# lxa9867/ImageFolder

Hardware: NVIDIA H100
Metric: tokenizer_train_images_per_sec_256x256 (higher is better)
Workload: dtype bf16

## Files before the change

imagefolder_b200/csrc/attn_kernel.cu:

```cuda
#include "xq_common.cuh"
#include "xq_tc.cuh"

namespace xq {
using namespace xqtc;

constexpr int AT_BM = 128;
constexpr int AT_BN = 128;
constexpr int AT_D = 64;
constexpr int AT_NS = 2;
constexpr int AT_TILE = AT_BM * AT_D * 2;
constexpr int AT_THREADS = 288;

struct AttnFwdSmem {
    static constexpr int Q = 0;
    static constexpr int K = AT_TILE;
    static constexpr int V = AT_TILE * (1 + AT_NS);
    static constexpr int BAR = AT_TILE * (1 + 2 * AT_NS);
    static constexpr int BYTES = BAR + 256;
};

__device__ __forceinline__ void named_bar_sync(int id, int nthreads) { asm volatile("bar.sync %0, %1;" ::"r"(id), "r"(nthreads) : "memory"); }

__global__ void __launch_bounds__(AT_THREADS, 1)
attn_fwd_kernel(const __grid_constant__ CUtensorMap tmQKV, __nv_bfloat16 *__restrict__ out, float *__restrict__ lse2, int N, int H,
                int nQ , float c ) {
    extern __shared__ uint8_t smem_raw[];
    uint8_t *base = (uint8_t *)(((uintptr_t)smem_raw + 1023) & ~(uintptr_t)1023);
    uint64_t *bars = (uint64_t *)(base + AttnFwdSmem::BAR);
    uint64_t *q_full = bars + 0;
    uint64_t *k_full = bars + 1;
    uint64_t *k_empty = bars + 1 + AT_NS;
    uint64_t *v_full = bars + 1 + 2 * AT_NS;
    uint64_t *v_empty = bars + 1 + 3 * AT_NS;

    const int tid = threadIdx.x, warp = tid >> 5, lane = tid & 31;
    const int nK = (N + AT_BN - 1) / AT_BN;
    const int bh = blockIdx.x / nQ, qt = blockIdx.x - bh * nQ;
    const int b = bh / H, h = bh - b * H;

    if (tid == 0) {
        mbar_init(q_full, 1);
        for (int i = 0; i < AT_NS; ++i) { mbar_init(&k_full[i], 1); mbar_init(&k_empty[i], 8); mbar_init(&v_full[i], 1); mbar_init(&v_empty[i], 8); }
        mbar_fence_init();
    }
    __syncthreads();

    if (warp == 8) {
        const int colQ = h * AT_D, colK = (H + h) * AT_D, colV = (2 * H + h) * AT_D;
        if (elect_one()) {
            tma_prefetch_desc(&tmQKV);
            mbar_expect_tx(q_full, AT_TILE);
            tma_load_3d(base + AttnFwdSmem::Q, &tmQKV, colQ, qt * AT_BM, b, q_full);
        }
        __syncwarp();
        for (int j = 0; j < nK; ++j) {
            const int st = j % AT_NS;
            const uint32_t ph = ((j / AT_NS) & 1) ^ 1;
            mbar_wait(&k_empty[st], ph);
            if (elect_one()) {
                mbar_expect_tx(&k_full[st], AT_TILE);
                tma_load_3d(base + AttnFwdSmem::K + st * AT_TILE, &tmQKV, colK, j * AT_BN, b, &k_full[st]);
            }
            __syncwarp();
            mbar_wait(&v_empty[st], ph);
            if (elect_one()) {
                mbar_expect_tx(&v_full[st], AT_TILE);
                tma_load_3d(base + AttnFwdSmem::V + st * AT_TILE, &tmQKV, colV, j * AT_BN, b, &v_full[st]);
            }
            __syncwarp();
        }
        return;
    }

    const int wg = warp >> 2, wq = warp & 3;
    const int rq = wg * 64 + wq * 16 + (lane >> 2), cq = 2 * (lane & 3);
    const uint64_t qd = desc_k_sw128(smem_u32(base + AttnFwdSmem::Q + wg * (AT_TILE / 2)));
    float m[2] = {-CUDART_INF_F, -CUDART_INF_F}, l[2] = {0.f, 0.f};
    float o[32];
#pragma unroll
    for (int i = 0; i < 32; ++i) o[i] = 0.f;
    mbar_wait(q_full, 0);
    for (int j = 0; j < nK; ++j) {
        const int st = j % AT_NS;
        const uint32_t ph = (j / AT_NS) & 1;
        float s[64];
        mbar_wait(&k_full[st], ph);
        const uint64_t kd = desc_k_sw128(smem_u32(base + AttnFwdSmem::K + st * AT_TILE));
        wgmma_fence();
#pragma unroll
        for (int k = 0; k < AT_D / 16; ++k) wgmma_m64n128k16_ss<0, 0>(s, desc_adv(qd, k * 32), desc_adv(kd, k * 32), (uint32_t)k);
        wgmma_commit();
        wgmma_wait<0>();
        fence_regs(s);
        __syncwarp();
        if (lane == 0) mbar_arrive(&k_empty[st]);
        const int nv = N - j * AT_BN;
        if (nv < AT_BN) {
#pragma unroll
            for (int i = 0; i < 64; ++i)
                if (8 * (i >> 2) + cq + (i & 1) >= nv) s[i] = -CUDART_INF_F;
        }
        float mx[2] = {m[0], m[1]};
#pragma unroll
        for (int i = 0; i < 64; ++i) mx[(i >> 1) & 1] = fmaxf(mx[(i >> 1) & 1], s[i]);
// ... 53 lines not shown

__global__ void __launch_bounds__(128)
attn_fwd_tail_kernel(const __nv_bfloat16 *__restrict__ qkv, __nv_bfloat16 *__restrict__ out, float *__restrict__ lse2, int B, int N,
                     int H, int n0 , float c) {
    const int lane = threadIdx.x & 31;
    const long long w = ((long long)blockIdx.x * blockDim.x + threadIdx.x) >> 5;
    const int nt = N - n0;
    if (w >= (long long)B * H * nt) return;
    const int r = (int)(w % nt);
    const int bh = (int)(w / nt);
    const int b = bh / H, h = bh - b * H;
    const int n = n0 + r;
    const size_t W = (size_t)3 * H * AT_D;
    const __nv_bfloat16 *qp = qkv + ((size_t)b * N + n) * W + h * AT_D;
    float qf[AT_D];
#pragma unroll
    for (int u = 0; u < 8; ++u) {
        const uint4 x = *reinterpret_cast<const uint4 *>(qp + u * 8);
        const __nv_bfloat162 *x2 = reinterpret_cast<const __nv_bfloat162 *>(&x);
#pragma unroll
        for (int e = 0; e < 4; ++e) {
            const float2 f = __bfloat1622float2(x2[e]);
            qf[u * 8 + 2 * e] = f.x * c;
            qf[u * 8 + 2 * e + 1] = f.y * c;
        }
    }
    float m = -CUDART_INF_F, l = 0.f, o[AT_D];
#pragma unroll
    for (int i = 0; i < AT_D; ++i) o[i] = 0.f;
    for (int key = lane; key < N; key += 32) {
        const __nv_bfloat16 *kp = qkv + ((size_t)b * N + key) * W + (H + h) * AT_D;
        const __nv_bfloat16 *vp = kp + (size_t)H * AT_D;
        float s = 0.f;
#pragma unroll
        for (int u = 0; u < 8; ++u) {
            const uint4 x = *reinterpret_cast<const uint4 *>(kp + u * 8);
            const __nv_bfloat162 *x2 = reinterpret_cast<const __nv_bfloat162 *>(&x);
#pragma unroll
            for (int e = 0; e < 4; ++e) {
                const float2 f = __bfloat1622float2(x2[e]);
                s = fmaf(qf[u * 8 + 2 * e], f.x, s);
                s = fmaf(qf[u * 8 + 2 * e + 1], f.y, s);
            }
        }
        const float m_new = fmaxf(m, s);
        const float corr = ex2_approx(m - m_new);
        const float p = ex2_approx(s - m_new);
        l = fmaf(l, corr, p);
        m = m_new;
#pragma unroll
        for (int u = 0; u < 8; ++u) {
            const uint4 x = *reinterpret_cast<const uint4 *>(vp + u * 8);
            const __nv_bfloat162 *x2 = reinterpret_cast<const __nv_bfloat162 *>(&x);
#pragma unroll
            for (int e = 0; e < 4; ++e) {
                const float2 f = __bfloat1622float2(x2[e]);
                o[u * 8 + 2 * e] = fmaf(o[u * 8 + 2 * e], corr, p * f.x);
                o[u * 8 + 2 * e + 1] = fmaf(o[u * 8 + 2 * e + 1], corr, p * f.y);
            }
        }
    }
    float M = m;
#pragma unroll
    for (int off = 16; off > 0; off >>= 1) M = fmaxf(M, __shfl_xor_sync(0xffffffffu, M, off));
    const float f = (m == -CUDART_INF_F) ? 0.f : ex2_approx(m - M);
    l *= f;
#pragma unroll
    for (int off = 16; off > 0; off >>= 1) l += __shfl_xor_sync(0xffffffffu, l, off);
    const float inv = 1.0f / l;
    float mine0 = 0.f, mine1 = 0.f;
#pragma unroll
    for (int i = 0; i < AT_D; ++i) {
        float x = o[i] * f;
#pragma unroll
        for (int off = 16; off > 0; off >>= 1) x += __shfl_xor_sync(0xffffffffu, x, off);
        if (i == 2 * lane) mine0 = x;
        if (i == 2 * lane + 1) mine1 = x;
    }
    __nv_bfloat16 *op = out + ((size_t)b * N + n) * H * AT_D + h * AT_D;
    *reinterpret_cast<uint32_t *>(op + 2 * lane) = pack_bf16(mine0 * inv, mine1 * inv);
    if (lane == 0) lse2[(size_t)bh * N + n] = M + log2f(l);
}

constexpr int AB_THREADS = 288;
constexpr int AB_BQ = 64;
constexpr int AB_QS = 3;
constexpr int AB_QTILE = AB_BQ * AT_D * 2;

struct AttnBwdSmem {
    static constexpr int K = 0;
    static constexpr int V = AT_TILE;
    static constexpr int Q = 2 * AT_TILE;
    static constexpr int DO = Q + AB_QS * AB_QTILE;
    static constexpr int DS = DO + AB_QS * AB_QTILE;
    static constexpr int STAT = DS + 2 * AB_QTILE;
    static constexpr int BAR = STAT + AB_QS * 512;
    static constexpr int BYTES = BAR + 256;
};

__device__ __forceinline__ void bwd_epilogue_frag(const float (&acc)[32], float mul, __nv_bfloat16 *__restrict__ row0,
                                                  size_t row_stride, bool ok0, bool ok1, float *__restrict__ g_bias_cols, int lane) {
    const int cq = 2 * (lane & 3);
#pragma unroll
    for (int jj = 0; jj < AT_D / 8; ++jj) {
        const uint32_t w0 = pack_bf16(acc[4 * jj] * mul, acc[4 * jj + 1] * mul);
        const uint32_t w1 = pack_bf16(acc[4 * jj + 2] * mul, acc[4 * jj + 3] * mul);
        if (ok0) *reinterpret_cast<uint32_t *>(row0 + 8 * jj + cq) = w0;
        if (ok1) *reinterpret_cast<uint32_t *>(row0 + 8 * row_stride + 8 * jj + cq) = w1;
        if (g_bias_cols) {
            float s0 = __uint_as_float(w0 << 16) + __uint_as_float(w1 << 16);
            float s1 = __uint_as_float(w0 & 0xffff0000u) + __uint_as_float(w1 & 0xffff0000u);
#pragma unroll
            for (int o = 4; o < 32; o <<= 1) {
                s0 += __shfl_xor_sync(0xffffffffu, s0, o);
                s1 += __shfl_xor_sync(0xffffffffu, s1, o);
            }
            if (lane < 4) {
                atomicAdd(g_bias_cols + 8 * jj + cq, s0);
                atomicAdd(g_bias_cols + 8 * jj + cq + 1, s1);
            }
        }
    }
}

__global__ void __launch_bounds__(AB_THREADS, 1)
attn_bwd_kernel(const __grid_constant__ CUtensorMap tmQKV, const __grid_constant__ CUtensorMap tmDO, const float *__restrict__ lseP,
                const float *__restrict__ deltaP, float *__restrict__ dq_acc, __nv_bfloat16 *__restrict__ dqkv, float *__restrict__ g_bias,
                int N, int H, int Npad, float c, float scale) {
    extern __shared__ uint8_t smem_raw[];
    uint8_t *base = (uint8_t *)(((uintptr_t)smem_raw + 1023) & ~(uintptr_t)1023);
    uint64_t *bars = (uint64_t *)(base + AttnBwdSmem::BAR);
    uint64_t *kv_full = bars;
    uint64_t *q_full = bars + 1;
    uint64_t *q_empty = bars + 1 + AB_QS;
    float *s_lse = (float *)(base + AttnBwdSmem::STAT);
    float *s_delta = s_lse + AB_QS * AB_BQ;

    const int tid = threadIdx.x, warp = tid >> 5, lane = tid & 31;
    const int bh = blockIdx.y, b = bh / H, h = bh - b * H;
    const int k0 = blockIdx.x * AT_BN;
    const int colQ = h * AT_D, colK = (H + h) * AT_D, colV = (2 * H + h) * AT_D;
    const int nQ = (N + AB_BQ - 1) / AB_BQ;

    if (tid == 0) {
        mbar_init(kv_full, 1);
        for (int i = 0; i < AB_QS; ++i) { mbar_init(&q_full[i], 1); mbar_init(&q_empty[i], 8); }
        mbar_fence_init();
    }
    __syncthreads();

    if (warp == 8) {
        if (elect_one()) {
            tma_prefetch_desc(&tmQKV);
            tma_prefetch_desc(&tmDO);
            mbar_expect_tx(kv_full, 2 * AT_TILE);
            for (int hf = 0; hf < 2; ++hf) {
                tma_load_3d(base + AttnBwdSmem::K + hf * AB_QTILE, &tmQKV, colK, k0 + hf * AB_BQ, b, kv_full);
                tma_load_3d(base + AttnBwdSmem::V + hf * AB_QTILE, &tmQKV, colV, k0 + hf * AB_BQ, b, kv_full);
            }
        }
        __syncwarp();
        for (int i = 0; i < nQ; ++i) {
            const int st = i % AB_QS;
            mbar_wait(&q_empty[st], ((i / AB_QS) & 1) ^ 1);
            if (elect_one()) {
                mbar_expect_tx(&q_full[st], 2 * AB_QTILE + 2 * AB_BQ * 4);
                tma_load_3d(base + AttnBwdSmem::Q + st * AB_QTILE, &tmQKV, colQ, i * AB_BQ, b, &q_full[st]);
                tma_load_3d(base + AttnBwdSmem::DO + st * AB_QTILE, &tmDO, h * AT_D, i * AB_BQ, b, &q_full[st]);
                bulk_g2s(s_lse + st * AB_BQ, lseP + (size_t)bh * Npad + i * AB_BQ, AB_BQ * 4, &q_full[st]);
                bulk_g2s(s_delta + st * AB_BQ, deltaP + (size_t)bh * Npad + i * AB_BQ, AB_BQ * 4, &q_full[st]);
            }
            __syncwarp();
        }
        return;
    }

    const int wg = warp >> 2, wq = warp & 3;
    const int rq = wq * 16 + (lane >> 2), cq = 2 * (lane & 3);
    const int key0 = k0 + wg * 64 + rq;
    const bool kok0 = key0 < N, kok1 = key0 + 8 < N;
    const uint32_t kw = smem_u32(base + AttnBwdSmem::K + wg * AB_QTILE), vw = smem_u32(base + AttnBwdSmem::V + wg * AB_QTILE);
    const uint64_t kd_k = desc_k_sw128(kw), vd_k = desc_k_sw128(vw), kd_mn = desc_mn_sw128(kw, AT_TILE);
    const uint32_t dsw = smem_u32(base + AttnBwdSmem::DS + wg * AB_QTILE);
    const uint64_t dsd = desc_mn_sw128(dsw, AT_TILE);
    float dv[32], dk[32];
#pragma unroll
    for (int i = 0; i < 32; ++i) dv[i] = dk[i] = 0.f;
    mbar_wait(kv_full, 0);
    for (int i = 0; i < nQ; ++i) {
        const int st = i % AB_QS;
        mbar_wait(&q_full[st], (i / AB_QS) & 1);
        const uint32_t qa = smem_u32(base + AttnBwdSmem::Q + st * AB_QTILE), da = smem_u32(base + AttnBwdSmem::DO + st * AB_QTILE);
        float s[32], dp[32];
        wgmma_fence();
#pragma unroll
        for (int k = 0; k < AT_D / 16; ++k) wgmma_m64n64k16_ss<0, 0>(s, desc_adv(kd_k, k * 32), desc_adv(desc_k_sw128(qa), k * 32), (uint32_t)k);
#pragma unroll
        for (int k = 0; k < AT_D / 16; ++k) wgmma_m64n64k16_ss<0, 0>(dp, desc_adv(vd_k, k * 32), desc_adv(desc_k_sw128(da), k * 32), (uint32_t)k);
        wgmma_commit();
        wgmma_wait<0>();
        fence_regs(s);
        fence_regs(dp);
        const float *L = s_lse + st * AB_BQ, *D = s_delta + st * AB_BQ;
        uint32_t pa[4][4], sa[4][4];
#pragma unroll
        for (int jj = 0; jj < AB_BQ / 8; ++jj) {
            const float2 Lq = *reinterpret_cast<const float2 *>(L + 8 * jj + cq);
            const float2 Dq = *reinterpret_cast<const float2 *>(D + 8 * jj + cq);
#pragma unroll
            for (int hh = 0; hh < 2; ++hh) {
                const bool ok = hh ? kok1 : kok0;
                const float p0 = ok ? ex2_approx(fmaf(s[4 * jj + 2 * hh], c, -Lq.x)) : 0.f;
                const float p1 = ok ? ex2_approx(fmaf(s[4 * jj + 2 * hh + 1], c, -Lq.y)) : 0.f;
                const uint32_t pw = pack_bf16(p0, p1);
                const float d0 = __uint_as_float(pw << 16) * (dp[4 * jj + 2 * hh] - Dq.x);
                const float d1 = __uint_as_float(pw & 0xffff0000u) * (dp[4 * jj + 2 * hh + 1] - Dq.y);
                const uint32_t dw = pack_bf16(d0, d1);
                pa[jj >> 1][(jj & 1) * 2 + hh] = pw;
                sa[jj >> 1][(jj & 1) * 2 + hh] = dw;
                asm volatile("st.shared.b32 [%0], %1;" ::"r"(dsw + rowtile_off_bf16(rq + 8 * hh, 8 * jj + cq)), "r"(dw) : "memory");
            }
        }
        fence_async_smem();
        named_bar_sync(1 + wg, 128);
        const uint64_t qd_mn = desc_mn_sw128(qa, AT_TILE), dd_mn = desc_mn_sw128(da, AT_TILE);
        float dq[32];
        wgmma_fence();
#pragma unroll
        for (int k = 0; k < AB_BQ / 16; ++k) {
            wgmma_m64n64k16_rs<1>(dv, pa[k], desc_adv(dd_mn, k * 2048), 1u);
            wgmma_m64n64k16_rs<1>(dk, sa[k], desc_adv(qd_mn, k * 2048), 1u);
        }
#pragma unroll
        for (int k = 0; k < 64 / 16; ++k) wgmma_m64n64k16_ss<1, 1>(dq, desc_adv(dsd, k * 2048), desc_adv(kd_mn, k * 2048), (uint32_t)k);
        wgmma_commit();
        wgmma_wait<0>();
        fence_regs(dv);
        fence_regs(dk);
        fence_regs(dq);
        __syncwarp();
        if (lane == 0) mbar_arrive(&q_empty[st]);
        named_bar_sync(1 + wg, 128);
#pragma unroll
        for (int hh = 0; hh < 2; ++hh) {
            const int q = i * AB_BQ + rq + 8 * hh;
            if (q < N) {
                float *dst = dq_acc + ((size_t)bh * N + q) * AT_D + cq;
#pragma unroll
                for (int jj = 0; jj < AT_D / 8; ++jj)
                    atomicAdd(reinterpret_cast<float2 *>(dst + 8 * jj), make_float2(dq[4 * jj + 2 * hh], dq[4 * jj + 2 * hh + 1]));
            }
        }
    }
    const size_t W = (size_t)3 * H * AT_D;
    __nv_bfloat16 *row = dqkv + ((size_t)b * N + key0) * W;
    bwd_epilogue_frag(dv, 1.0f, row + colV, W, kok0, kok1, g_bias ? g_bias + colV : nullptr, lane);
    bwd_epilogue_frag(dk, scale, row + colK, W, kok0, kok1, g_bias ? g_bias + colK : nullptr, lane);
}


constexpr int AB_KTAIL_MAX = 4;
constexpr int AB_PREP_ROWS = 128;

__device__ __forceinline__ void unpack8(const uint4 &w, float (&f)[8]) {
    const uint32_t x[4] = {w.x, w.y, w.z, w.w};
#pragma unroll
    for (int e = 0; e < 4; ++e) { f[2 * e] = __uint_as_float(x[e] << 16); f[2 * e + 1] = __uint_as_float(x[e] & 0xffff0000u); }
}

template <int NT>
__global__ void __launch_bounds__(256, 2)
attn_bwd_prep_kernel(const __nv_bfloat16 *__restrict__ qkv, const __nv_bfloat16 *__restrict__ out, const __nv_bfloat16 *__restrict__ dout,
                     const float *__restrict__ lse2, float *__restrict__ lseP, float *__restrict__ deltaP, float *__restrict__ dq_acc,
                     float *__restrict__ dsT, __nv_bfloat16 *__restrict__ dqkv, float *__restrict__ g_bias, int N, int H, int Npad,
                     float c, float scale) {
    constexpr int NTA = NT > 0 ? NT : 1;
    __shared__ float red[NT > 0 ? 8 : 1][2][NTA][AT_D];
    __shared__ __align__(16) float skv[2][NTA][AT_D];
    const int bh = blockIdx.y, b = bh / H, h = bh - b * H;
    const int lane = threadIdx.x & 31, sub = threadIdx.x & 7, rloc = threadIdx.x >> 3;
    const int n0 = N - NT;
    const size_t W = (size_t)3 * H * AT_D;
    const __nv_bfloat16 *qb = qkv + (size_t)b * N * W + h * AT_D + sub * 8;
    const size_t ob = (size_t)b * N * H * AT_D + h * AT_D + sub * 8;
    float aK[NTA][8], aV[NTA][8];
    if constexpr (NT > 0) {
        if (threadIdx.x < NT * 16) {
            const int t = threadIdx.x >> 4, isv = (threadIdx.x >> 3) & 1;
            float f[8];
            unpack8(*reinterpret_cast<const uint4 *>(qb + (size_t)(n0 + t) * W + (size_t)(1 + isv) * H * AT_D), f);
#pragma unroll
            for (int e = 0; e < 8; ++e) skv[isv][t][sub * 8 + e] = f[e];
        }
#pragma unroll
        for (int t = 0; t < NT; ++t) {
#pragma unroll
            for (int e = 0; e < 8; ++e) aK[t][e] = aV[t][e] = 0.f;
        }
        __syncthreads();
    }
    constexpr int PASSES = AB_PREP_ROWS / 32;
    extern __shared__ uint4 prep_stage[];
    auto prefetch = [&](int blk, int stg) {
#pragma unroll
        for (int ps = 0; ps < PASSES; ++ps) {
            const int n = blk * AB_PREP_ROWS + ps * 32 + rloc;
            const int nc = n < N ? n : N - 1;
            uint4 *dst = prep_stage + ((size_t)(stg * 3) * PASSES + ps) * 256 + threadIdx.x;
            cp_async16(dst, out + ob + (size_t)nc * H * AT_D);
            cp_async16(dst + PASSES * 256, dout + ob + (size_t)nc * H * AT_D);
            cp_async16(dst + 2 * PASSES * 256, qb + (size_t)nc * W);
        }
        cp_async_commit();
    };
    if constexpr (NT > 0) prefetch(blockIdx.x, 0);
    int stg = 0;
    for (int blk = blockIdx.x; blk * AB_PREP_ROWS < Npad; blk += gridDim.x, stg ^= 1) {
        uint4 ow[PASSES], gw[PASSES], qw[PASSES];
        float lq[PASSES];
#pragma unroll
        for (int ps = 0; ps < PASSES; ++ps) {
            const int n = blk * AB_PREP_ROWS + ps * 32 + rloc;
            const int nc = n < N ? n : N - 1;
            if constexpr (NT == 0) {
                ow[ps] = *reinterpret_cast<const uint4 *>(out + ob + (size_t)nc * H * AT_D);
                gw[ps] = *reinterpret_cast<const uint4 *>(dout + ob + (size_t)nc * H * AT_D);
            }
            lq[ps] = lse2[(size_t)bh * N + nc];
        }
        if constexpr (NT > 0) {
            if ((blk + (int)gridDim.x) * AB_PREP_ROWS < Npad) { prefetch(blk + gridDim.x, stg ^ 1); cp_async_wait<1>(); }
            else cp_async_wait<0>();
        }
#pragma unroll
        for (int ps = 0; ps < PASSES; ++ps) {
            const int n = blk * AB_PREP_ROWS + ps * 32 + rloc;
// ... 109 lines not shown
    for (int e = 0; e < 8; ++e) v[e] = 0.f;
#pragma unroll
    for (int ps = 0; ps < PASSES; ++ps) {
        const int n = blockIdx.x * AB_CONV_ROWS + ps * 32 + rloc;
        if (n < N) {
            const size_t rowid = (size_t)bhh * N + n;
            float x[8] = {x0[ps].x, x0[ps].y, x0[ps].z, x0[ps].w, x1[ps].x, x1[ps].y, x1[ps].z, x1[ps].w};
            for (int t = 0; t < nt; ++t) {
                const float ds = dsT[rowid * nt + t];
#pragma unroll
                for (int e = 0; e < 8; ++e) x[e] = fmaf(ds, skt[t][part * 8 + e], x[e]);
            }
            uint4 o;
            o.x = pack_bf16(x[0] * scale, x[1] * scale);
            o.y = pack_bf16(x[2] * scale, x[3] * scale);
            o.z = pack_bf16(x[4] * scale, x[5] * scale);
            o.w = pack_bf16(x[6] * scale, x[7] * scale);
            *reinterpret_cast<uint4 *>(dqkv + (((size_t)bb * N + n) * 3 * H + hh) * AT_D + part * 8) = o;
            const uint32_t w[4] = {o.x, o.y, o.z, o.w};
#pragma unroll
            for (int e = 0; e < 4; ++e) { v[2 * e] += __uint_as_float(w[e] << 16); v[2 * e + 1] += __uint_as_float(w[e] & 0xffff0000u); }
        }
    }
    if (!g_bias) return;
#pragma unroll
    for (int e = 0; e < 8; ++e) {
        v[e] += __shfl_xor_sync(0xffffffffu, v[e], 8);
        v[e] += __shfl_xor_sync(0xffffffffu, v[e], 16);
    }
    const int warp = threadIdx.x >> 5, lane = threadIdx.x & 31;
    if (lane < 8) {
#pragma unroll
        for (int e = 0; e < 8; ++e) red[warp][lane * 8 + e] = v[e];
    }
    __syncthreads();
    if (threadIdx.x < AT_D) {
        float acc = 0.f;
#pragma unroll
        for (int w8 = 0; w8 < 8; ++w8) acc += red[w8][threadIdx.x];
        atomicAdd(g_bias + hh * AT_D + threadIdx.x, acc);
    }
}

static int attn_bwd_ktail(int N) {
    const int r = N % AT_BN;
    return (N > AT_BN && r != 0 && r <= AB_KTAIL_MAX) ? r : 0;
}

static size_t attn_bwd_ws_layout(int B, int N, int H, size_t *off_lse, size_t *off_delta, size_t *off_dst) {
    const size_t Npad = ((size_t)N + AT_BM - 1) / AT_BM * AT_BM;
    const size_t acc = align_up((size_t)B * H * N * AT_D * sizeof(float), 1024);
    const size_t st = align_up((size_t)B * H * Npad * sizeof(float), 1024);
    const size_t dst = align_up((size_t)B * H * N * attn_bwd_ktail(N) * sizeof(float), 1024);
    if (off_lse) *off_lse = acc;
    if (off_delta) *off_delta = acc + st;
    if (off_dst) *off_dst = acc + 2 * st;
    return acc + 2 * st + dst;
}

}

extern "C" {

size_t xq_vit_attn_bwd_workspace_bytes(int B, int N, int H) {
    if (B <= 0 || N <= 0 || H <= 0) return 0;
    return xq::attn_bwd_ws_layout(B, N, H, nullptr, nullptr, nullptr);
}

int xq_vit_attn_bwd(const void *qkv, const void *out, const void *d_out, const float *lse2, void *dqkv, float *g_bias, int B, int N,
                    int H, int head_dim, float scale, void *workspace, size_t workspace_bytes, void *stream) {
    using namespace xq;
    if (!qkv || !out || !d_out || !lse2 || !dqkv || !workspace || B <= 0 || N <= 0 || H <= 0) return XQ_ERR_ARG;
    if (head_dim != AT_D) return XQ_ERR_UNSUPPORTED;
    if (((uintptr_t)qkv & 15) || ((uintptr_t)out & 15) || ((uintptr_t)d_out & 15) || ((uintptr_t)dqkv & 15) || ((uintptr_t)workspace & 255))
        return XQ_ERR_ARG;
    size_t off_lse, off_delta, off_dst;
    if (workspace_bytes < attn_bwd_ws_layout(B, N, H, &off_lse, &off_delta, &off_dst)) return XQ_ERR_WORKSPACE;
    cudaStream_t st = (cudaStream_t)stream;
    float *acc = (float *)workspace;
    float *lseP = (float *)((char *)workspace + off_lse);
    float *deltaP = (float *)((char *)workspace + off_delta);
    float *dsT = (float *)((char *)workspace + off_dst);
    const uint64_t W = (uint64_t)3 * H * AT_D, Wo = (uint64_t)H * AT_D;
    CUtensorMap tmQKV, tmDO;
    if (!tensor_map_bf16_3d(&tmQKV, qkv, W, N, B, W * 2, (uint64_t)N * W * 2, AB_BQ) ||
        !tensor_map_bf16_3d(&tmDO, d_out, Wo, N, B, Wo * 2, (uint64_t)N * Wo * 2, AB_BQ))
        return XQ_ERR_UNSUPPORTED;
    const int nt = attn_bwd_ktail(N);
    const int nK = nt ? N / AT_BN : (N + AT_BN - 1) / AT_BN;
    const int Npad = (N + AT_BM - 1) / AT_BM * AT_BM;
    if ((long long)B * H > 65535) return XQ_ERR_UNSUPPORTED;
    if (g_bias) XQ_CUDA_TRY(cudaMemsetAsync(g_bias, 0, (size_t)3 * H * AT_D * sizeof(float), st));
    const float c2 = scale * 1.4426950408889634f;
    {
        dim3 grid(nt ? 1u : (unsigned)(Npad / AB_PREP_ROWS), (unsigned)(B * H));
        const size_t ps = nt ? (size_t)2 * 3 * (AB_PREP_ROWS / 32) * 256 * 16 : 0;
        decltype(&attn_bwd_prep_kernel<0>) const preps[] = {attn_bwd_prep_kernel<0>, attn_bwd_prep_kernel<1>, attn_bwd_prep_kernel<2>,
                                                            attn_bwd_prep_kernel<3>, attn_bwd_prep_kernel<4>};
        const auto prep = preps[nt < 4 ? nt : 4];
        if (int rc = smem_optin(prep, ps)) return rc;
        prep<<<grid, 256, ps, st>>>((const __nv_bfloat16 *)qkv, (const __nv_bfloat16 *)out, (const __nv_bfloat16 *)d_out, lse2, lseP,
                                    deltaP, acc, dsT, (__nv_bfloat16 *)dqkv, g_bias, N, H, Npad, c2, scale);
        XQ_LAUNCH_CHECK("attn_bwd_prep_kernel");
    }
    const size_t smem = AttnBwdSmem::BYTES + 1024;
    if (int rc = smem_optin(attn_bwd_kernel, smem)) return rc;
    attn_bwd_kernel<<<dim3((unsigned)nK, (unsigned)(B * H)), AB_THREADS, smem, st>>>(tmQKV, tmDO, lseP, deltaP, acc,
                                                                                     (__nv_bfloat16 *)dqkv, g_bias, N, H, Npad, c2, scale);
    XQ_LAUNCH_CHECK("attn_bwd_kernel");
    {
        dim3 grid((unsigned)((N + AB_CONV_ROWS - 1) / AB_CONV_ROWS), (unsigned)(B * H));
        attn_dq_convert_kernel<<<grid, 256, 0, st>>>(acc, (const __nv_bfloat16 *)qkv, dsT, (__nv_bfloat16 *)dqkv, g_bias, N, H, N - nt, nt, scale);
        XQ_LAUNCH_CHECK("attn_dq_convert_kernel");
    }
    return XQ_OK;
}

int xq_vit_attn_fwd(const void *qkv, void *out, float *lse2, int B, int N, int H, int head_dim, float scale, void *stream) {
    using namespace xq;
    if (!qkv || !out || !lse2 || B <= 0 || N <= 0 || H <= 0) return XQ_ERR_ARG;
    if (head_dim != AT_D) return XQ_ERR_UNSUPPORTED;
    if (((uintptr_t)qkv & 15) || ((uintptr_t)out & 15)) return XQ_ERR_ARG;
    const uint64_t W = (uint64_t)3 * H * AT_D;
    CUtensorMap tmQKV;
    if (!tensor_map_bf16_3d(&tmQKV, qkv, W, N, B, W * 2, (uint64_t)N * W * 2, AT_BM)) return XQ_ERR_UNSUPPORTED;
    const int n_tail = (N % AT_BM != 0 && N % AT_BM <= AT_TAIL_MAX && N > AT_BM) ? N % AT_BM : 0;
    const int nQ = n_tail ? N / AT_BM : (N + AT_BM - 1) / AT_BM;
    const size_t smem = AttnFwdSmem::BYTES + 1024;
    if (int rc = smem_optin(attn_fwd_kernel, smem)) return rc;
    const long long tiles = (long long)B * H * nQ;
    if (tiles > 0x7fffffffLL) return XQ_ERR_ARG;
    const float c = scale * 1.4426950408889634f;
    attn_fwd_kernel<<<(unsigned)tiles, AT_THREADS, smem, (cudaStream_t)stream>>>(tmQKV, (__nv_bfloat16 *)out, lse2, N, H, nQ, c);
    XQ_LAUNCH_CHECK("attn_fwd_kernel");
    if (n_tail) {
        const long long warps = (long long)B * H * n_tail;
        attn_fwd_tail_kernel<<<(unsigned)((warps + 3) / 4), 128, 0, (cudaStream_t)stream>>>(
            (const __nv_bfloat16 *)qkv, (__nv_bfloat16 *)out, lse2, B, N, H, N - n_tail, c);
        XQ_LAUNCH_CHECK("attn_fwd_tail_kernel");
    }
    return XQ_OK;
}

}
```

imagefolder_b200/csrc/xq_tc.cuh:

```cuda
#pragma once
#include <cuda.h>
#include <cuda_bf16.h>
#include <cuda_runtime.h>
#include <stdint.h>

#include <cstring>
#include <mutex>

namespace xqtc {

__device__ __forceinline__ uint32_t smem_u32(const void *p) { return (uint32_t)__cvta_generic_to_shared(p); }

__device__ __forceinline__ void mbar_init(uint64_t *bar, uint32_t count) {
    asm volatile("mbarrier.init.shared::cta.b64 [%0], %1;" ::"r"(smem_u32(bar)), "r"(count));
}
__device__ __forceinline__ void mbar_fence_init() { asm volatile("fence.mbarrier_init.release.cluster;" ::: "memory"); }
__device__ __forceinline__ void mbar_expect_tx(uint64_t *bar, uint32_t bytes) {
    asm volatile("mbarrier.arrive.expect_tx.shared::cta.b64 _, [%0], %1;" ::"r"(smem_u32(bar)), "r"(bytes) : "memory");
}
__device__ __forceinline__ void mbar_arrive(uint64_t *bar) {
    asm volatile("mbarrier.arrive.shared::cta.b64 _, [%0];" ::"r"(smem_u32(bar)) : "memory");
}
__device__ __forceinline__ bool mbar_test(uint64_t *bar, uint32_t parity) {
    uint32_t done;
    asm volatile(
        "{\n\t.reg .pred p;\n\t"
        "mbarrier.test_wait.parity.shared::cta.b64 p, [%1], %2;\n\t"
        "selp.b32 %0, 1, 0, p;\n\t}"
        : "=r"(done)
        : "r"(smem_u32(bar)), "r"(parity)
        : "memory");
    return done != 0;
}
__device__ __forceinline__ bool mbar_try(uint64_t *bar, uint32_t parity) {
    uint32_t done;
    asm volatile(
        "{\n\t.reg .pred p;\n\t"
        "mbarrier.try_wait.parity.shared::cta.b64 p, [%1], %2;\n\t"
        "selp.b32 %0, 1, 0, p;\n\t}"
        : "=r"(done)
        : "r"(smem_u32(bar)), "r"(parity)
        : "memory");
    return done != 0;
}
__device__ __forceinline__ void mbar_wait(uint64_t *bar, uint32_t parity) {
    while (!mbar_try(bar, parity)) {}
}
__device__ __forceinline__ void mbar_wait_ptx(uint64_t *bar, uint32_t parity) {
    asm volatile(
        "{\n\t.reg .pred p;\n\tXQ_MBAR_WAIT:\n\t"
        "mbarrier.try_wait.parity.shared::cta.b64 p, [%0], %1;\n\t"
        "@p bra XQ_MBAR_DONE;\n\tbra XQ_MBAR_WAIT;\n\tXQ_MBAR_DONE:\n\t}" ::"r"(smem_u32(bar)), "r"(parity) : "memory");
}

__device__ __forceinline__ void tma_prefetch_desc(const CUtensorMap *map) {
    asm volatile("prefetch.tensormap [%0];" ::"l"(reinterpret_cast<uint64_t>(map)) : "memory");
}
__device__ __forceinline__ void bulk_g2s(void *dst, const void *src, uint32_t bytes, uint64_t *bar) {
    asm volatile("cp.async.bulk.shared::cluster.global.mbarrier::complete_tx::bytes [%0], [%1], %2, [%3];"
                 ::"r"(smem_u32(dst)), "l"(src), "r"(bytes), "r"(smem_u32(bar))
                 : "memory");
}
__device__ __forceinline__ void tma_load_2d(void *dst, const CUtensorMap *map, int c0, int c1, uint64_t *bar) {
    asm volatile(
        "cp.async.bulk.tensor.2d.shared::cluster.global.mbarrier::complete_tx::bytes [%0], [%1, {%2, %3}], [%4];"
        ::"r"(smem_u32(dst)), "l"(reinterpret_cast<uint64_t>(map)), "r"(c0), "r"(c1), "r"(smem_u32(bar))
        : "memory");
}
__device__ __forceinline__ void tma_load_3d(void *dst, const CUtensorMap *map, int c0, int c1, int c2, uint64_t *bar) {
    asm volatile(
        "cp.async.bulk.tensor.3d.shared::cluster.global.mbarrier::complete_tx::bytes [%0], [%1, {%2, %3, %4}], [%5];"
        ::"r"(smem_u32(dst)), "l"(reinterpret_cast<uint64_t>(map)), "r"(c0), "r"(c1), "r"(c2), "r"(smem_u32(bar))
        : "memory");
}
__device__ __forceinline__ void tma_store_3d(const CUtensorMap *map, const void *src, int c0, int c1, int c2) {
    asm volatile("cp.async.bulk.tensor.3d.global.shared::cta.bulk_group [%0, {%2, %3, %4}], [%1];"
                 ::"l"(reinterpret_cast<uint64_t>(map)), "r"(smem_u32(src)), "r"(c0), "r"(c1), "r"(c2)
                 : "memory");
}
__device__ __forceinline__ void tma_reduce_add_3d(const CUtensorMap *map, const void *src, int c0, int c1, int c2) {
    asm volatile("cp.reduce.async.bulk.tensor.3d.global.shared::cta.add.tile.bulk_group [%0, {%2, %3, %4}], [%1];"
                 ::"l"(reinterpret_cast<uint64_t>(map)), "r"(smem_u32(src)), "r"(c0), "r"(c1), "r"(c2)
                 : "memory");
}
__device__ __forceinline__ void bulk_commit() { asm volatile("cp.async.bulk.commit_group;" ::: "memory"); }
template <int N>
__device__ __forceinline__ void bulk_wait_read() { asm volatile("cp.async.bulk.wait_group.read %0;" ::"n"(N) : "memory"); }
template <int N>
__device__ __forceinline__ void bulk_wait() { asm volatile("cp.async.bulk.wait_group %0;" ::"n"(N) : "memory"); }

__device__ __forceinline__ void fence_async_smem() { asm volatile("fence.proxy.async.shared::cta;" ::: "memory"); }

__device__ __forceinline__ uint64_t desc_k_sw128(uint32_t smem_addr) {
    uint64_t d = 0;
    d |= (uint64_t)((smem_addr & 0x3FFFFu) >> 4);
    d |= (uint64_t)1 << 16;
    d |= (uint64_t)(1024 >> 4) << 32;
    d |= (uint64_t)1 << 62;
    return d;
}
__device__ __forceinline__ uint64_t desc_mn_sw128(uint32_t smem_addr, uint32_t lbo_bytes) {
    uint64_t d = 0;
    d |= (uint64_t)((smem_addr & 0x3FFFFu) >> 4);
    d |= (uint64_t)((lbo_bytes >> 4) & 0x3FFFu) << 16;
    d |= (uint64_t)(1024 >> 4) << 32;
    d |= (uint64_t)1 << 62;
    return d;
}
__device__ __forceinline__ uint64_t desc_adv(uint64_t d, uint32_t bytes) { return d + (uint64_t)(bytes >> 4); }

__device__ __forceinline__ void wgmma_fence() { asm volatile("wgmma.fence.sync.aligned;" ::: "memory"); }
__device__ __forceinline__ void wgmma_commit() { asm volatile("wgmma.commit_group.sync.aligned;" ::: "memory"); }
template <int N>
__device__ __forceinline__ void wgmma_wait() { asm volatile("wgmma.wait_group.sync.aligned %0;" ::"n"(N) : "memory"); }
template <int N>
__device__ __forceinline__ void fence_regs(float (&d)[N]) {
#pragma unroll
    for (int i = 0; i < N; ++i) asm volatile("" : "+f"(d[i])::"memory");
}

template <int TA, int TB>
__device__ __forceinline__ void wgmma_m64n64k16_ss(float (&d)[32], uint64_t da, uint64_t db, uint32_t acc) {
    asm volatile(
        "{\n\t.reg .pred p;\n\tsetp.ne.b32 p, %34, 0;\n\t"
        "wgmma.mma_async.sync.aligned.m64n64k16.f32.bf16.bf16 "
        "{%0, %1, %2, %3, %4, %5, %6, %7, %8, %9, %10, %11, %12, %13, %14, %15, %16, %17, %18, %19, %20, %21, %22, %23, %24, %25, %26, %27, %28, %29, %30, %31}, %32, %33, p, 1, 1, %35, %36;\n\t}"
        : "+f"(d[0]), "+f"(d[1]), "+f"(d[2]), "+f"(d[3]), "+f"(d[4]), "+f"(d[5]), "+f"(d[6]), "+f"(d[7]), "+f"(d[8]), "+f"(d[9]), "+f"(d[10]), "+f"(d[11]), "+f"(d[12]), "+f"(d[13]), "+f"(d[14]), "+f"(d[15]), "+f"(d[16]), "+f"(d[17]), "+f"(d[18]), "+f"(d[19]), "+f"(d[20]), "+f"(d[21]), "+f"(d[22]), "+f"(d[23]), "+f"(d[24]), "+f"(d[25]), "+f"(d[26]), "+f"(d[27]), "+f"(d[28]), "+f"(d[29]), "+f"(d[30]), "+f"(d[31])
        : "l"(da), "l"(db), "r"(acc), "n"(TA), "n"(TB));
}

template <int TA, int TB>
__device__ __forceinline__ void wgmma_m64n128k16_ss(float (&d)[64], uint64_t da, uint64_t db, uint32_t acc) {
    asm volatile(
        "{\n\t.reg .pred p;\n\tsetp.ne.b32 p, %66, 0;\n\t"
        "wgmma.mma_async.sync.aligned.m64n128k16.f32.bf16.bf16 "
        "{%0, %1, %2, %3, %4, %5, %6, %7, %8, %9, %10, %11, %12, %13, %14, %15, %16, %17, %18, %19, %20, %21, %22, %23, %24, %25, %26, %27, %28, %29, %30, %31, %32, %33, %34, %35, %36, %37, %38, %39, %40, %41, %42, %43, %44, %45, %46, %47, %48, %49, %50, %51, %52, %53, %54, %55, %56, %57, %58, %59, %60, %61, %62, %63}, %64, %65, p, 1, 1, %67, %68;\n\t}"
        : "+f"(d[0]), "+f"(d[1]), "+f"(d[2]), "+f"(d[3]), "+f"(d[4]), "+f"(d[5]), "+f"(d[6]), "+f"(d[7]), "+f"(d[8]), "+f"(d[9]), "+f"(d[10]), "+f"(d[11]), "+f"(d[12]), "+f"(d[13]), "+f"(d[14]), "+f"(d[15]), "+f"(d[16]), "+f"(d[17]), "+f"(d[18]), "+f"(d[19]), "+f"(d[20]), "+f"(d[21]), "+f"(d[22]), "+f"(d[23]), "+f"(d[24]), "+f"(d[25]), "+f"(d[26]), "+f"(d[27]), "+f"(d[28]), "+f"(d[29]), "+f"(d[30]), "+f"(d[31]), "+f"(d[32]), "+f"(d[33]), "+f"(d[34]), "+f"(d[35]), "+f"(d[36]), "+f"(d[37]), "+f"(d[38]), "+f"(d[39]), "+f"(d[40]), "+f"(d[41]), "+f"(d[42]), "+f"(d[43]), "+f"(d[44]), "+f"(d[45]), "+f"(d[46]), "+f"(d[47]), "+f"(d[48]), "+f"(d[49]), "+f"(d[50]), "+f"(d[51]), "+f"(d[52]), "+f"(d[53]), "+f"(d[54]), "+f"(d[55]), "+f"(d[56]), "+f"(d[57]), "+f"(d[58]), "+f"(d[59]), "+f"(d[60]), "+f"(d[61]), "+f"(d[62]), "+f"(d[63])
        : "l"(da), "l"(db), "r"(acc), "n"(TA), "n"(TB));
}

template <int TB>
__device__ __forceinline__ void wgmma_m64n64k16_rs(float (&d)[32], const uint32_t (&a)[4], uint64_t db, uint32_t acc) {
    asm volatile(
        "{\n\t.reg .pred p;\n\tsetp.ne.b32 p, %37, 0;\n\t"
        "wgmma.mma_async.sync.aligned.m64n64k16.f32.bf16.bf16 "
        "{%0, %1, %2, %3, %4, %5, %6, %7, %8, %9, %10, %11, %12, %13, %14, %15, %16, %17, %18, %19, %20, %21, %22, %23, %24, %25, %26, %27, %28, %29, %30, %31}, {%32, %33, %34, %35}, %36, p, 1, 1, %38;\n\t}"
        : "+f"(d[0]), "+f"(d[1]), "+f"(d[2]), "+f"(d[3]), "+f"(d[4]), "+f"(d[5]), "+f"(d[6]), "+f"(d[7]), "+f"(d[8]), "+f"(d[9]), "+f"(d[10]), "+f"(d[11]), "+f"(d[12]), "+f"(d[13]), "+f"(d[14]), "+f"(d[15]), "+f"(d[16]), "+f"(d[17]), "+f"(d[18]), "+f"(d[19]), "+f"(d[20]), "+f"(d[21]), "+f"(d[22]), "+f"(d[23]), "+f"(d[24]), "+f"(d[25]), "+f"(d[26]), "+f"(d[27]), "+f"(d[28]), "+f"(d[29]), "+f"(d[30]), "+f"(d[31])
        : "r"(a[0]), "r"(a[1]), "r"(a[2]), "r"(a[3]), "l"(db), "r"(acc), "n"(TB));
}

__device__ __forceinline__ void wgmma_m64n128k8_tf32(float (&d)[64], uint64_t da, uint64_t db, uint32_t acc) {
    asm volatile(
        "{\n\t.reg .pred p;\n\tsetp.ne.b32 p, %66, 0;\n\t"
        "wgmma.mma_async.sync.aligned.m64n128k8.f32.tf32.tf32 "
        "{%0, %1, %2, %3, %4, %5, %6, %7, %8, %9, %10, %11, %12, %13, %14, %15, %16, %17, %18, %19, %20, %21, %22, %23, %24, %25, %26, %27, %28, %29, %30, %31, %32, %33, %34, %35, %36, %37, %38, %39, %40, %41, %42, %43, %44, %45, %46, %47, %48, %49, %50, %51, %52, %53, %54, %55, %56, %57, %58, %59, %60, %61, %62, %63}, %64, %65, p, 1, 1;\n\t}"
        : "+f"(d[0]), "+f"(d[1]), "+f"(d[2]), "+f"(d[3]), "+f"(d[4]), "+f"(d[5]), "+f"(d[6]), "+f"(d[7]), "+f"(d[8]), "+f"(d[9]), "+f"(d[10]), "+f"(d[11]), "+f"(d[12]), "+f"(d[13]), "+f"(d[14]), "+f"(d[15]), "+f"(d[16]), "+f"(d[17]), "+f"(d[18]), "+f"(d[19]), "+f"(d[20]), "+f"(d[21]), "+f"(d[22]), "+f"(d[23]), "+f"(d[24]), "+f"(d[25]), "+f"(d[26]), "+f"(d[27]), "+f"(d[28]), "+f"(d[29]), "+f"(d[30]), "+f"(d[31]), "+f"(d[32]), "+f"(d[33]), "+f"(d[34]), "+f"(d[35]), "+f"(d[36]), "+f"(d[37]), "+f"(d[38]), "+f"(d[39]), "+f"(d[40]), "+f"(d[41]), "+f"(d[42]), "+f"(d[43]), "+f"(d[44]), "+f"(d[45]), "+f"(d[46]), "+f"(d[47]), "+f"(d[48]), "+f"(d[49]), "+f"(d[50]), "+f"(d[51]), "+f"(d[52]), "+f"(d[53]), "+f"(d[54]), "+f"(d[55]), "+f"(d[56]), "+f"(d[57]), "+f"(d[58]), "+f"(d[59]), "+f"(d[60]), "+f"(d[61]), "+f"(d[62]), "+f"(d[63])
        : "l"(da), "l"(db), "r"(acc));
}

__device__ __forceinline__ void sts128(uint32_t saddr, uint4 v) {
    asm volatile("st.shared.v4.b32 [%0], {%1, %2, %3, %4};" ::"r"(saddr), "r"(v.x), "r"(v.y), "r"(v.z), "r"(v.w) : "memory");
}
__device__ __forceinline__ float4 lds128f(uint32_t saddr) {
    float4 v;
    asm volatile("ld.shared.v4.f32 {%0, %1, %2, %3}, [%4];" : "=f"(v.x), "=f"(v.y), "=f"(v.z), "=f"(v.w) : "r"(saddr) : "memory");
    return v;
}

__device__ __forceinline__ bool elect_one() {
    uint32_t pred;
    asm volatile("{\n\t.reg .pred P;\n\telect.sync _|P, 0xffffffff;\n\tselp.b32 %0, 1, 0, P;\n\t}" : "=r"(pred));
    return pred != 0;
}

__host__ __device__ __forceinline__ uint32_t rowtile_off_bf16(int r, int c) {
    return (uint32_t)(r * 128 + ((((c >> 3) ^ (r & 7)) & 7) << 4) + (c & 7) * 2);
}
__host__ __device__ __forceinline__ uint32_t rowtile_unit(int r, int u) { return (uint32_t)(r * 128 + ((u ^ (r & 7)) << 4)); }

__device__ __forceinline__ uint32_t pack_bf16(float lo, float hi) {
    uint32_t r;
    asm("cvt.rn.bf16x2.f32 %0, %1, %2;" : "=r"(r) : "f"(hi), "f"(lo));
    return r;
}
__device__ __forceinline__ float ex2_approx(float x) {
    float y;
    asm("ex2.approx.ftz.f32 %0, %1;" : "=f"(y) : "f"(x));
    return y;
}

constexpr int TMAP_CACHE = 128;

inline bool tensor_map(CUtensorMap *out, const void *base, CUtensorMapDataType dtype, int rank, const cuuint64_t *dims,
                       const cuuint64_t *strides, const cuuint32_t *box, CUtensorMapSwizzle swizzle) {
    typedef CUresult (*Encode)(CUtensorMap *, CUtensorMapDataType, cuuint32_t, void *, const cuuint64_t *, const cuuint64_t *,
                               const cuuint32_t *, const cuuint32_t *, CUtensorMapInterleave, CUtensorMapSwizzle,
                               CUtensorMapL2promotion, CUtensorMapFloatOOBfill);
    struct Entry { uint64_t key[12]; CUtensorMap map; };
    static std::mutex mu;
    static Entry cache[TMAP_CACHE];
    static int n_cached = 0, next = 0;
    static Encode encode = nullptr;
    if (rank < 1 || rank > 3) return false;
    uint64_t key[12] = {(uint64_t)(uintptr_t)base, (uint64_t)dtype, (uint64_t)rank, (uint64_t)swizzle};
    for (int i = 0; i < rank; ++i) { key[4 + i] = dims[i]; key[7 + i] = box[i]; }
    for (int i = 0; i + 1 < rank; ++i) key[10 + i] = strides[i];
    std::lock_guard<std::mutex> g(mu);
    for (int i = 0; i < n_cached; ++i)
        if (memcmp(cache[i].key, key, sizeof(key)) == 0) { *out = cache[i].map; return true; }
    if (!encode) {
// ... 29 lines not shown
```

Baseline: 581.4.

## Reduce dQ in shared memory and push via TMA reduce-add in attention backward

The attention backward kernel used to accumulate dQ with per-element float2 global atomics from each warpgroup. It now sums the two warpgroups' dQ tiles into a double-buffered swizzled shared tile and issues TMA bulk reduce-add stores, using named barriers for the handoff. The dK/dV MMAs are also reordered after dQ so they can overlap the reduction. A narrow N=16 path handles a short final query block, and register reallocation with an extra producer warpgroup is added. This adds shared memory and synchronization complexity in exchange for far fewer global atomics.

```diff
diff --git a/imagefolder_b200/csrc/attn_kernel.cu b/imagefolder_b200/csrc/attn_kernel.cu
--- a/imagefolder_b200/csrc/attn_kernel.cu
+++ b/imagefolder_b200/csrc/attn_kernel.cu
@@ -1,3 +1,5 @@
+#include <type_traits>
+
 #include "xq_common.cuh"
 #include "xq_tc.cuh"
 
@@ -18,8 +20,6 @@
     static constexpr int BAR = AT_TILE * (1 + 2 * AT_NS);
     static constexpr int BYTES = BAR + 256;
 };
-
-__device__ __forceinline__ void named_bar_sync(int id, int nthreads) { asm volatile("bar.sync %0, %1;" ::"r"(id), "r"(nthreads) : "memory"); }
 
 __global__ void __launch_bounds__(AT_THREADS, 1)
 attn_fwd_kernel(const __grid_constant__ CUtensorMap tmQKV, __nv_bfloat16 *__restrict__ out, float *__restrict__ lse2, int N, int H,
@@ -239,10 +239,13 @@
     if (lane == 0) lse2[(size_t)bh * N + n] = M + log2f(l);
 }
 
-constexpr int AB_THREADS = 288;
+constexpr int AB_THREADS = 384;
 constexpr int AB_BQ = 64;
 constexpr int AB_QS = 3;
 constexpr int AB_QTILE = AB_BQ * AT_D * 2;
+constexpr int AB_DQTILE = AB_BQ * AT_D * 4;
+constexpr int AB_BAR_DQ_FULL = 3;
+constexpr int AB_BAR_DQ_FREE = 4;
 
 struct AttnBwdSmem {
     static constexpr int K = 0;
@@ -250,10 +253,15 @@
     static constexpr int Q = 2 * AT_TILE;
     static constexpr int DO = Q + AB_QS * AB_QTILE;
     static constexpr int DS = DO + AB_QS * AB_QTILE;
-    static constexpr int STAT = DS + 2 * AB_QTILE;
+    static constexpr int DQ = DS + 2 * AB_QTILE;
+    static constexpr int STAT = DQ + 2 * AB_DQTILE;
     static constexpr int BAR = STAT + AB_QS * 512;
     static constexpr int BYTES = BAR + 256;
 };
+
+__device__ __forceinline__ uint32_t dq_tile_off(int r, int c) {
+    return (uint32_t)((c >> 5) * (AB_DQTILE / 2) + r * 128 + ((((c & 31) >> 2) ^ (r & 7)) << 4) + (c & 3) * 4);
+}
 
 __device__ __forceinline__ void bwd_epilogue_frag(const float (&acc)[32], float mul, __nv_bfloat16 *__restrict__ row0,
                                                   size_t row_stride, bool ok0, bool ok1, float *__restrict__ g_bias_cols, int lane) {
@@ -282,8 +290,8 @@
 
 __global__ void __launch_bounds__(AB_THREADS, 1)
 attn_bwd_kernel(const __grid_constant__ CUtensorMap tmQKV, const __grid_constant__ CUtensorMap tmDO, const float *__restrict__ lseP,
-                const float *__restrict__ deltaP, float *__restrict__ dq_acc, __nv_bfloat16 *__restrict__ dqkv, float *__restrict__ g_bias,
-                int N, int H, int Npad, float c, float scale) {
+                const float *__restrict__ deltaP, const __grid_constant__ CUtensorMap tmDQ, __nv_bfloat16 *__restrict__ dqkv,
+                float *__restrict__ g_bias, int N, int H, int Npad, float c, float scale) {
     extern __shared__ uint8_t smem_raw[];
     uint8_t *base = (uint8_t *)(((uintptr_t)smem_raw + 1023) & ~(uintptr_t)1023);
     uint64_t *bars = (uint64_t *)(base + AttnBwdSmem::BAR);
@@ -306,10 +314,13 @@
     }
     __syncthreads();
 
-    if (warp == 8) {
+    if (warp >= 8) {
+        setmaxnreg_dec<24>();
+        if (warp != 8) return;
         if (elect_one()) {
             tma_prefetch_desc(&tmQKV);
             tma_prefetch_desc(&tmDO);
+            tma_prefetch_desc(&tmDQ);
             mbar_expect_tx(kv_full, 2 * AT_TILE);
             for (int hf = 0; hf < 2; ++hf) {
                 tma_load_3d(base + AttnBwdSmem::K + hf * AB_QTILE, &tmQKV, colK, k0 + hf * AB_BQ, b, kv_full);
@@ -332,6 +343,7 @@
         return;
     }
 
+    setmaxnreg_inc<240>();
     const int wg = warp >> 2, wq = warp & 3;
     const int rq = wq * 16 + (lane >> 2), cq = 2 * (lane & 3);
     const int key0 = k0 + wg * 64 + rq;
@@ -343,17 +355,29 @@
     float dv[32], dk[32];
 #pragma unroll
     for (int i = 0; i < 32; ++i) dv[i] = dk[i] = 0.f;
+    const uint32_t dqs = smem_u32(base + AttnBwdSmem::DQ);
+    if (wg == 1) named_bar_arrive(AB_BAR_DQ_FREE, 256);
     mbar_wait(kv_full, 0);
-    for (int i = 0; i < nQ; ++i) {
+    auto query_block = [&](int i, auto narrow_tag) {
+        constexpr bool NARROW = decltype(narrow_tag)::value;
         const int st = i % AB_QS;
         mbar_wait(&q_full[st], (i / AB_QS) & 1);
         const uint32_t qa = smem_u32(base + AttnBwdSmem::Q + st * AB_QTILE), da = smem_u32(base + AttnBwdSmem::DO + st * AB_QTILE);
         float s[32], dp[32];
         wgmma_fence();
-#pragma unroll
-        for (int k = 0; k < AT_D / 16; ++k) wgmma_m64n64k16_ss<0, 0>(s, desc_adv(kd_k, k * 32), desc_adv(desc_k_sw128(qa), k * 32), (uint32_t)k);
-#pragma unroll
-        for (int k = 0; k < AT_D / 16; ++k) wgmma_m64n64k16_ss<0, 0>(dp, desc_adv(vd_k, k * 32), desc_adv(desc_k_sw128(da), k * 32), (uint32_t)k);
+        if constexpr (NARROW) {
+            float(&s16)[8] = *reinterpret_cast<float(*)[8]>(s);
+            float(&dp16)[8] = *reinterpret_cast<float(*)[8]>(dp);
+#pragma unroll
+            for (int k = 0; k < AT_D / 16; ++k) wgmma_m64n16k16_ss<0, 0>(s16, desc_adv(kd_k, k * 32), desc_adv(desc_k_sw128(qa), k * 32), (uint32_t)k);
+#pragma unroll
+            for (int k = 0; k < AT_D / 16; ++k) wgmma_m64n16k16_ss<0, 0>(dp16, desc_adv(vd_k, k * 32), desc_adv(desc_k_sw128(da), k * 32), (uint32_t)k);
+        } else {
+#pragma unroll
+            for (int k = 0; k < AT_D / 16; ++k) wgmma_m64n64k16_ss<0, 0>(s, desc_adv(kd_k, k * 32), desc_adv(desc_k_sw128(qa), k * 32), (uint32_t)k);
+#pragma unroll
+            for (int k = 0; k < AT_D / 16; ++k) wgmma_m64n64k16_ss<0, 0>(dp, desc_adv(vd_k, k * 32), desc_adv(desc_k_sw128(da), k * 32), (uint32_t)k);
+        }
         wgmma_commit();
         wgmma_wait<0>();
         fence_regs(s);
@@ -362,6 +386,7 @@
         uint32_t pa[4][4], sa[4][4];
 #pragma unroll
         for (int jj = 0; jj < AB_BQ / 8; ++jj) {
+            if (NARROW && jj >= 2) continue;
             const float2 Lq = *reinterpret_cast<const float2 *>(L + 8 * jj + cq);
             const float2 Dq = *reinterpret_cast<const float2 *>(D + 8 * jj + cq);
 #pragma unroll
@@ -384,31 +409,63 @@
         float dq[32];
         wgmma_fence();
 #pragma unroll
-        for (int k = 0; k < AB_BQ / 16; ++k) {
-            wgmma_m64n64k16_rs<1>(dv, pa[k], desc_adv(dd_mn, k * 2048), 1u);
-            wgmma_m64n64k16_rs<1>(dk, sa[k], desc_adv(qd_mn, k * 2048), 1u);
-        }
-#pragma unroll
         for (int k = 0; k < 64 / 16; ++k) wgmma_m64n64k16_ss<1, 1>(dq, desc_adv(dsd, k * 2048), desc_adv(kd_mn, k * 2048), (uint32_t)k);
         wgmma_commit();
+        wgmma_m64n64k16_rs<1>(dv, pa[0], dd_mn, 1u);
+        wgmma_m64n64k16_rs<1>(dk, sa[0], qd_mn, 1u);
+        if constexpr (!NARROW) {
+#pragma unroll
+            for (int k = 1; k < AB_BQ / 16; ++k) {
+                wgmma_m64n64k16_rs<1>(dv, pa[k], desc_adv(dd_mn, k * 2048), 1u);
+                wgmma_m64n64k16_rs<1>(dk, sa[k], desc_adv(qd_mn, k * 2048), 1u);
+            }
+        }
+        wgmma_commit();
+        wgmma_wait<1>();
+        fence_regs(dq);
+        named_bar_sync(1 + wg, 128);
+        const uint32_t dqt = dqs + (i & 1) * AB_DQTILE;
+        if (wg == 0) named_bar_sync(AB_BAR_DQ_FREE, 256);
+        else named_bar_sync(AB_BAR_DQ_FULL, 256);
+#pragma unroll
+        for (int hh = 0; hh < 2; ++hh) {
+#pragma unroll
+            for (int jj = 0; jj < AT_D / 8; ++jj) {
+                const uint32_t a = dqt + dq_tile_off(rq + 8 * hh, 8 * jj + cq);
+                float x0 = dq[4 * jj + 2 * hh], x1 = dq[4 * jj + 2 * hh + 1];
+                if (wg == 1) {
+                    float y0, y1;
+                    asm volatile("ld.shared.v2.f32 {%0, %1}, [%2];" : "=f"(y0), "=f"(y1) : "r"(a) : "memory");
+                    x0 += y0;
+                    x1 += y1;
+                }
+                asm volatile("st.shared.v2.f32 [%0], {%1, %2};" ::"r"(a), "f"(x0), "f"(x1) : "memory");
+            }
+        }
+        if (wg == 0) {
+            named_bar_arrive(AB_BAR_DQ_FULL, 256);
+        } else {
+            fence_async_smem();
+            named_bar_sync(2, 128);
+            if (tid == 128) {
+                tma_reduce_add_3d(&tmDQ, base + AttnBwdSmem::DQ + (i & 1) * AB_DQTILE, 0, i * AB_BQ, bh);
+                tma_reduce_add_3d(&tmDQ, base + AttnBwdSmem::DQ + (i & 1) * AB_DQTILE + AB_DQTILE / 2, 32, i * AB_BQ, bh);
+                bulk_commit();
+                bulk_wait_read<1>();
+            }
+            __syncwarp();
+            if (i + 1 < nQ) named_bar_arrive(AB_BAR_DQ_FREE, 256);
+        }
         wgmma_wait<0>();
         fence_regs(dv);
         fence_regs(dk);
-        fence_regs(dq);
         __syncwarp();
         if (lane == 0) mbar_arrive(&q_empty[st]);
-        named_bar_sync(1 + wg, 128);
-#pragma unroll
-        for (int hh = 0; hh < 2; ++hh) {
-            const int q = i * AB_BQ + rq + 8 * hh;
-            if (q < N) {
-                float *dst = dq_acc + ((size_t)bh * N + q) * AT_D + cq;
-#pragma unroll
-                for (int jj = 0; jj < AT_D / 8; ++jj)
-                    atomicAdd(reinterpret_cast<float2 *>(dst + 8 * jj), make_float2(dq[4 * jj + 2 * hh], dq[4 * jj + 2 * hh + 1]));
-            }
-        }
-    }
+    };
+    const bool narrow_last = N - (nQ - 1) * AB_BQ <= 16;
+    for (int i = 0; i < nQ - (narrow_last ? 1 : 0); ++i) query_block(i, std::false_type{});
+    if (narrow_last) query_block(nQ - 1, std::true_type{});
+    if (tid == 128) bulk_wait<0>();
     const size_t W = (size_t)3 * H * AT_D;
     __nv_bfloat16 *row = dqkv + ((size_t)b * N + key0) * W;
     bwd_epilogue_frag(dv, 1.0f, row + colV, W, kok0, kok1, g_bias ? g_bias + colV : nullptr, lane);
@@ -684,9 +741,13 @@
     float *deltaP = (float *)((char *)workspace + off_delta);
     float *dsT = (float *)((char *)workspace + off_dst);
     const uint64_t W = (uint64_t)3 * H * AT_D, Wo = (uint64_t)H * AT_D;
-    CUtensorMap tmQKV, tmDO;
+    CUtensorMap tmQKV, tmDO, tmDQ;
+    const cuuint64_t dq_dims[3] = {(cuuint64_t)AT_D, (cuuint64_t)N, (cuuint64_t)B * H};
+    const cuuint64_t dq_strides[2] = {(cuuint64_t)AT_D * 4, (cuuint64_t)N * AT_D * 4};
+    const cuuint32_t dq_box[3] = {32u, (cuuint32_t)AB_BQ, 1u};
     if (!tensor_map_bf16_3d(&tmQKV, qkv, W, N, B, W * 2, (uint64_t)N * W * 2, AB_BQ) ||
-        !tensor_map_bf16_3d(&tmDO, d_out, Wo, N, B, Wo * 2, (uint64_t)N * Wo * 2, AB_BQ))
+        !tensor_map_bf16_3d(&tmDO, d_out, Wo, N, B, Wo * 2, (uint64_t)N * Wo * 2, AB_BQ) ||
+        !tensor_map(&tmDQ, acc, CU_TENSOR_MAP_DATA_TYPE_FLOAT32, 3, dq_dims, dq_strides, dq_box, CU_TENSOR_MAP_SWIZZLE_128B))
         return XQ_ERR_UNSUPPORTED;
     const int nt = attn_bwd_ktail(N);
     const int nK = nt ? N / AT_BN : (N + AT_BN - 1) / AT_BN;
@@ -707,7 +768,7 @@
     }
     const size_t smem = AttnBwdSmem::BYTES + 1024;
     if (int rc = smem_optin(attn_bwd_kernel, smem)) return rc;
-    attn_bwd_kernel<<<dim3((unsigned)nK, (unsigned)(B * H)), AB_THREADS, smem, st>>>(tmQKV, tmDO, lseP, deltaP, acc,
+    attn_bwd_kernel<<<dim3((unsigned)nK, (unsigned)(B * H)), AB_THREADS, smem, st>>>(tmQKV, tmDO, lseP, deltaP, tmDQ,
                                                                                      (__nv_bfloat16 *)dqkv, g_bias, N, H, Npad, c2, scale);
     XQ_LAUNCH_CHECK("attn_bwd_kernel");
     {
diff --git a/imagefolder_b200/csrc/xq_tc.cuh b/imagefolder_b200/csrc/xq_tc.cuh
--- a/imagefolder_b200/csrc/xq_tc.cuh
+++ b/imagefolder_b200/csrc/xq_tc.cuh
@@ -90,6 +90,13 @@
 __device__ __forceinline__ void bulk_wait() { asm volatile("cp.async.bulk.wait_group %0;" ::"n"(N) : "memory"); }
 
 __device__ __forceinline__ void fence_async_smem() { asm volatile("fence.proxy.async.shared::cta;" ::: "memory"); }
+
+__device__ __forceinline__ void named_bar_sync(int id, int nthreads) { asm volatile("bar.sync %0, %1;" ::"r"(id), "r"(nthreads) : "memory"); }
+__device__ __forceinline__ void named_bar_arrive(int id, int nthreads) { asm volatile("bar.arrive %0, %1;" ::"r"(id), "r"(nthreads) : "memory"); }
+template <int R>
+__device__ __forceinline__ void setmaxnreg_inc() { asm volatile("setmaxnreg.inc.sync.aligned.u32 %0;" ::"n"(R)); }
+template <int R>
+__device__ __forceinline__ void setmaxnreg_dec() { asm volatile("setmaxnreg.dec.sync.aligned.u32 %0;" ::"n"(R)); }
 
 __device__ __forceinline__ uint64_t desc_k_sw128(uint32_t smem_addr) {
     uint64_t d = 0;
@@ -126,6 +133,16 @@
         "wgmma.mma_async.sync.aligned.m64n64k16.f32.bf16.bf16 "
         "{%0, %1, %2, %3, %4, %5, %6, %7, %8, %9, %10, %11, %12, %13, %14, %15, %16, %17, %18, %19, %20, %21, %22, %23, %24, %25, %26, %27, %28, %29, %30, %31}, %32, %33, p, 1, 1, %35, %36;\n\t}"
         : "+f"(d[0]), "+f"(d[1]), "+f"(d[2]), "+f"(d[3]), "+f"(d[4]), "+f"(d[5]), "+f"(d[6]), "+f"(d[7]), "+f"(d[8]), "+f"(d[9]), "+f"(d[10]), "+f"(d[11]), "+f"(d[12]), "+f"(d[13]), "+f"(d[14]), "+f"(d[15]), "+f"(d[16]), "+f"(d[17]), "+f"(d[18]), "+f"(d[19]), "+f"(d[20]), "+f"(d[21]), "+f"(d[22]), "+f"(d[23]), "+f"(d[24]), "+f"(d[25]), "+f"(d[26]), "+f"(d[27]), "+f"(d[28]), "+f"(d[29]), "+f"(d[30]), "+f"(d[31])
+        : "l"(da), "l"(db), "r"(acc), "n"(TA), "n"(TB));
+}
+
+template <int TA, int TB>
+__device__ __forceinline__ void wgmma_m64n16k16_ss(float (&d)[8], uint64_t da, uint64_t db, uint32_t acc) {
+    asm volatile(
+        "{\n\t.reg .pred p;\n\tsetp.ne.b32 p, %10, 0;\n\t"
+        "wgmma.mma_async.sync.aligned.m64n16k16.f32.bf16.bf16 "
+        "{%0, %1, %2, %3, %4, %5, %6, %7}, %8, %9, p, 1, 1, %11, %12;\n\t}"
+        : "+f"(d[0]), "+f"(d[1]), "+f"(d[2]), "+f"(d[3]), "+f"(d[4]), "+f"(d[5]), "+f"(d[6]), "+f"(d[7])
         : "l"(da), "l"(db), "r"(acc), "n"(TA), "n"(TB));
 }
 
```

New measurement: 597.2, median of 6. 2.7% higher.
